# maropu/hivemall

Measured on AMD Instinct MI355X. Metric: rows/sec (node) FFM on Criteo-shaped sparse at 1/2/4/8 MI355X; logloss parity, higher is better.
Workload: dtype fp32; 1 GPU; global_batch=262144, seq_len=39, nnz_per_row=39, fields=explicit, parallelism=dp1, mix_every=10, state=fp32 V, fp32 AdaGrad accumulator per (feature, field) slot (fp32 math), state_layout=packed, reload=False, mixed_bytes_per_mix=671088656, mix_overlapped=False, mix_wire=bf16_delta, early_ramp_warmup_steps=1, linear_steps=side-table, resident_batches=8

## Files before the change

csrc/kernels/ffm.hip:

```cpp
#include <type_traits>

#include "common.h"

namespace {

struct FFMParams {
    int B, F;
    int num_features, num_fields, Kp;
    int classification;
    int train;
    int use_linear, use_bias, norm;
    int reload;
    int gstride;
    int vpad;
    int tail16;
    int gfstride;
    int sstride;
    int fstride;
    long long vfe;
    uint32_t seed;
    float eta0, eps, lambda_v;
    float alpha, beta, lambda1, lambda2;
    float min_target, max_target;
    const uint8_t* hot;
// ... 791 lines not shown
            defer_row(P, row);
        } else if (P.train) {
            const float ks = kappa * scale * scale;
            const f2 eps = {P.eps, P.eps};
            const f2 meta = {-P.eta0, -P.eta0};
            uint32_t hrow = (P.seed ^ ((uint32_t)row * 0x85EBCA77u)) + tid_h;
            hrow ^= hrow >> 16;
            hrow *= 0x7FEB352Du;
            hrow ^= hrow >> 15;
#pragma unroll
            for (int j = 0; j < NS; ++j) {
                const int s = tid + j * 256;
                const f2 coef = {ks * xab[j], ks * xab[j]};
                f2 o0, o1, g0, g1, p0, p1;
                if constexpr (BF) {
                    const uint2 pv = s_t[s < FF ? s : 0];
                    o0 = bf2_to_f2(q[j].x); o1 = bf2_to_f2(q[j].y);
                    g0 = bf2_to_f2(q[j].z); g1 = bf2_to_f2(q[j].w);
                    p0 = bf2_to_f2(pv.x);   p1 = bf2_to_f2(pv.y);
                } else {
                    const float4 pv = s_t[s < FF ? s : 0];
                    o0 = f2{qv[j].x, qv[j].y}; o1 = f2{qv[j].z, qv[j].w};
                    g0 = f2{qg[j].x, qg[j].y}; g1 = f2{qg[j].z, qg[j].w};
                    p0 = f2{pv.x, pv.y};       p1 = f2{pv.z, pv.w};
                }
                const float lj = (live >> j & 1u) ? P.lambda_v : 0.f;
                const f2 lamj = {lj, lj};
                const f2 d0 = coef * p0 + lamj * o0, d1 = coef * p1 + lamj * o1;
                g0 = g0 + d0 * d0;
                g1 = g1 + d1 * d1;
                const f2 t0 = g0 + eps, t1 = g1 + eps;
                const f2 r0 = {__builtin_amdgcn_rsqf(t0.x), __builtin_amdgcn_rsqf(t0.y)};
                const f2 r1 = {__builtin_amdgcn_rsqf(t1.x), __builtin_amdgcn_rsqf(t1.y)};
                o0 = o0 + meta * d0 * r0;
                o1 = o1 + meta * d1 * r1;
                if constexpr (!BF) {
                    if (wr >> j & 1u) {
                        *reinterpret_cast<float4*>(vg + off[j]) = make_float4(o0.x, o0.y, o1.x, o1.y);
                        *reinterpret_cast<float4*>(vg + off[j] + 16u) = make_float4(g0.x, g0.y, g1.x, g1.y);
                    }
                    continue;
                }
                const uint32_t h = rotl32(hrow, 5 * j + 1) ^ (0x9E3779B9u * (uint32_t)(j + 1));
                const uint4 st = make_uint4(pack_sr_hi(o0, h, rotl32(h, 16)),
                                            pack_sr_hi(o1, rotl32(h, 8), rotl32(h, 24)),
                                            pack_sr_hi(g0, rotl32(h, 4), rotl32(h, 20)),
                                            pack_sr_hi(g1, rotl32(h, 12), rotl32(h, 28)));
                if (wr >> j & 1u) *reinterpret_cast<uint4*>(vg + off[j]) = st;
            }
            if (wave == 0 && lane < F) {
                const int pi = s_m[cur][lane].x;
                if (pi >= 0) {
                    for (int f = P.num_fields; f < (int)nfld; ++f) {
                        *reinterpret_cast<uint4*>(vg + ((uint32_t)pi * nfld + (uint32_t)f) * SLOT_B) = make_uint4(0u, 0u, 0u, 0u);
                        if (!BF) *reinterpret_cast<uint4*>(vg + ((uint32_t)pi * nfld + (uint32_t)f) * SLOT_B + 16u) = make_uint4(0u, 0u, 0u, 0u);
                    }
                }
            }
            if (mi >= 0) {
                if (P.use_linear) {
                    const float lz = s_lin[cur][1][lane];
                    const float ln = s_lin[cur][2][lane];
                    const float g = kappa * mx * scale;
                    const float n1 = ln + g * g;
                    const float z1 = lz + g - (sqrtf(n1) - sqrtf(ln)) / P.alpha * lw;
                    LW(wz, mi) = z1;
                    LW(wn, mi) = n1;
                    LW(w, mi) = ftrl_weight(z1, n1, P.alpha, P.beta, P.lambda1, P.lambda2);
                }
            }
            if (P.use_bias && tid == 0) bias_update(P, kappa, bias);
        }
        if (more) dma_lin(nxt);
    }
    __builtin_amdgcn_s_waitcnt(0x0F70);
#undef SA
#undef SB
}


typedef uint32_t u3v_t __attribute__((ext_vector_type(3)));

#define VMCNT_ENC(n) ((((n) & 15) | (((n) >> 4) << 14)) | 0x0F70)
template <int NS, typename OT, int TPB = 256, int ATOM = 0, int KV = 1, int KEEP = 0, int LT = 0>
__global__ __launch_bounds__(TPB) __attribute__((amdgpu_waves_per_eu(TPB / 128))) void ffm_pipe_sg32_kernel(
    FFMParams P, const int32_t* __restrict__ idx, const int32_t* __restrict__ fld,
    const float* __restrict__ val, const float* __restrict__ y, void* __restrict__ Vt,
    float* __restrict__ Gt, float* __restrict__ w, float* __restrict__ wz, float* __restrict__ wn,
    float* __restrict__ bias, float* __restrict__ pred_out, float* __restrict__ loss_out)
{
    __shared__ __attribute__((aligned(16))) float4 s_rv[NS * TPB * KV];
    __shared__ __attribute__((aligned(16))) float s_rg[NS * TPB];
    __shared__ __attribute__((aligned(16))) float4 s_t[NS * TPB * KV];
    __shared__ __attribute__((aligned(16))) int4 s_m[2][48];
    __shared__ __attribute__((aligned(16))) int s_mr[2][3][48];
    __shared__ __attribute__((aligned(16))) float s_lin[2][3][48];
    __shared__ __attribute__((aligned(16))) float4 s_lin4[2][48];
    __shared__ float s_red[TPB / 64 + 2];
    __shared__ int s_rep[TPB / 64];
    __shared__ float s_bias[4];
    __shared__ float s_bcur[2];
    __shared__ float2 s_hd[LT ? HD_SIZE : 1];
    __shared__ __attribute__((aligned(16))) float4 s_hacc[LT ? 2 : 1][48];
    __shared__ __attribute__((aligned(16))) int s_nh[LT ? 2 : 1][48];
    const int F = P.F;
    const int FF = F * F;
    const int tid = threadIdx.x, wave = tid >> 6, lane = tid & 63;
    constexpr int W_META = 1, W_LIN = 2, W_DMA = 3;
    const OT vfs = (OT)P.fstride * (16u * KV);
    const OT gfs = (OT)P.gstride * 4u;
    const int G = (int)gridDim.x;
    const int bid = (int)blockIdx.x;
    char* vb = reinterpret_cast<char*>(Vt);
    char* gb = reinterpret_cast<char*>(Gt);
    const bool latom = ATOM == 0 && !LT && P.lin_atomic == 1 && G > 1;
    if constexpr (LT != 0) {
        for (int t = tid; t < HD_SIZE; t += TPB) s_hd[t] = make_float2(0.f, 0.f);
    }
    int nh = -1, kh = -1;

    int ab[NS];
#pragma unroll
    for (int j = 0; j < NS; ++j) {
        const int s = tid + j * TPB;
        ab[j] = s < FF ? (s / F) | ((s % F) << 8) : 0;
    }
#define SA(j) (ab[j] & 0xFF)
#define SB(j) (ab[j] >> 8)

    auto dma_meta = [&](int bf, int row) {
        if (wave == W_DMA && lane < F && row < P.B) {
            const size_t o = (size_t)row * F + lane;
            __builtin_amdgcn_global_load_lds((glb_ptr_t)(idx + o), (lds_ptr_t)&s_mr[bf][0][0], 4, 0, 0);
            if (fld) __builtin_amdgcn_global_load_lds((glb_ptr_t)(fld + o), (lds_ptr_t)&s_mr[bf][1][0], 4, 0, 0);
            if (val) __builtin_amdgcn_global_load_lds((glb_ptr_t)(val + o), (lds_ptr_t)&s_mr[bf][2][0], 4, 0, 0);
        }
    };
    auto publish_meta = [&](int bf) {
        if (wave == W_META) {
            float sq = 0.f;
            if (lane < F) {
                int ri = s_mr[bf][0][lane];
                int rf = fld ? s_mr[bf][1][lane] : lane;
                float rx = val ? __int_as_float(s_mr[bf][2][lane]) : 1.f;
                if (ri < 0 || ri >= P.num_features || rf < 0 || rf >= P.num_fields) { ri = -1; rx = 0.f; rf = 0; }
                const int hb = ((ATOM == 2 || (latom && P.lin_atomic >= 2)) && ri >= 0) ? (int)P.hot[ri] : 0;
                s_m[bf][lane] = make_int4(ri, rf, __float_as_int(rx), hb);
                sq = rx * rx;
            }
            const float tot = hm::wave_sum_uniform(sq);
            if (lane == 0) s_red[TPB / 64 + bf] = (P.norm && tot > 0.f) ? rsqrtf(tot) : 1.f;
        }
    };
    auto slot = [&](int bf, int j, OT& ov, OT& og, float& xab) -> uint32_t {
        const int4 ma = s_m[bf][SA(j)], mb = s_m[bf][SB(j)];
        const bool ok = (ma.x | mb.x) >= 0 && tid + j * TPB < FF;
        const bool live = ok && SA(j) != SB(j);
        const OT i = ok ? (OT)(uint32_t)ma.x : (OT)0, f = ok ? (OT)(uint32_t)mb.y : (OT)0;
        ov = i * vfs + f * (16u * KV);
        og = i * gfs + f * 4u;
        xab = live ? __int_as_float(ma.z) * __int_as_float(mb.z) : 0.f;
        return live ? 1u : (ok ? 2u : 0u);
    };
    OT kov[KEEP ? NS : 1], kog[KEEP ? NS : 1], nov[KEEP ? NS : 1], nog[KEEP ? NS : 1];
    float kxab[KEEP ? NS : 1], nxab[KEEP ? NS : 1];
    uint32_t klive = 0u, kwr = 0u, nlive = 0u, nwr = 0u;
    int krep = 0, nrep = 0;
    auto dma_slots = [&](int bf) {
        if constexpr (KEEP) { nlive = 0u; nwr = 0u; nrep = 0; }
#pragma unroll
        for (int j = 0; j < NS; ++j) {
            OT ov, og;
            float xab;
            const uint32_t k = slot(bf, j, ov, og, xab);
            if constexpr (KEEP) {
                nov[j] = ov;
                nog[j] = og;
                nxab[j] = xab;
                nlive |= (k & 1u) << j;
                nwr |= (uint32_t)(k != 0u) << j;
                if (P.defer) nrep |= (int)slot_repeats(SA(j), SB(j), s_m[bf][SA(j)], s_m[bf][SB(j)]);
            }
#pragma unroll
            for (int q = 0; q < KV; ++q)
                __builtin_amdgcn_global_load_lds((glb_ptr_t)(vb + ov + 16u * q),
                                                 (lds_ptr_t)(s_rv + (q * NS + j) * TPB + wave * 64), 16, 0, 0);
            __builtin_amdgcn_global_load_lds((glb_ptr_t)(gb + og), (lds_ptr_t)(s_rg + j * TPB + wave * 64), 4, 0, 0);
        }
    };
    auto keep_rotate = [&]() {
        if constexpr (KEEP) {
#pragma unroll
            for (int j = 0; j < NS; ++j) { kov[j] = nov[j]; kog[j] = nog[j]; kxab[j] = nxab[j]; }
            klive = nlive; kwr = nwr; krep = nrep;
        }
    };
    const int nlin = (P.use_linear && P.lin_defer) ? ((P.lpack || !P.train) ? 1 + (LT != 0) : 3) : 0;
    auto dma_lin = [&](int bf) {
        if (P.use_linear && wave == W_LIN && lane < F) {
            const int i = max(s_m[bf][lane].x, 0);
            if (P.lpack) {
                __builtin_amdgcn_global_load_lds((glb_ptr_t)&LW(w, i), (lds_ptr_t)&s_lin4[bf][0], 16, 0, 0);
                if constexpr (LT != 0)
                    __builtin_amdgcn_global_load_lds((glb_ptr_t)(P.hacc + HACC_STRIDE * max(nh, 0)), (lds_ptr_t)&s_hacc[bf][0], 16, 0, 0);
                return;
            }
            __builtin_amdgcn_global_load_lds((glb_ptr_t)&LW(w, i), (lds_ptr_t)&s_lin[bf][0][0], 4, 0, 0);
            if (P.train) {
                __builtin_amdgcn_global_load_lds((glb_ptr_t)&LW(wz, i), (lds_ptr_t)&s_lin[bf][1][0], 4, 0, 0);
                __builtin_amdgcn_global_load_lds((glb_ptr_t)&LW(wn, i), (lds_ptr_t)&s_lin[bf][2][0], 4, 0, 0);
            }
        }
    };

    int row = bid;
    if (row >= P.B) return;
    if (tid == 0) { s_bcur[0] = 0.f; s_bcur[1] = 0.f; }
    dma_meta(0, row);
    __builtin_amdgcn_s_waitcnt(0x0F70);
    bar_raw();
    publish_meta(0);
    bar_raw();
    dma_slots(0);
    keep_rotate();
    if constexpr (LT != 0) {
        if (wave == W_LIN && lane < F) nh = s_m[0][lane].x >= 0 ? P.hidx[s_m[0][lane].x] : -1;
    }
    dma_lin(0);
    kh = nh;
    dma_meta(1, row + G);

    float4 fv[NS][KV];
    float fg[NS];
    OT fo[NS];
    uint32_t fwd = 0u;
    const bool bsh = P.use_bias && P.bias_sh;
    int bit = 0;
    float bz = 0.f, bn = 0.f;
    if (bsh && wave == W_META && lane < P.bias_s) {
        bz = __hip_atomic_load(P.bias_sh + lane * 32, __ATOMIC_RELAXED, __HIP_MEMORY_SCOPE_AGENT);
        bn = __hip_atomic_load(P.bias_sh + lane * 32 + 1, __ATOMIC_RELAXED, __HIP_MEMORY_SCOPE_AGENT);
    }
    for (int cur = 0; row < P.B; row += G, cur ^= 1) {
        const int nxt = cur ^ 1;
        const bool more = row + G < P.B;
        if (wave == W_LIN && nlin == 3) __builtin_amdgcn_s_waitcnt(0x0F73);
        else if (wave == W_LIN && nlin == 2) __builtin_amdgcn_s_waitcnt(0x0F72);
        else if (wave == W_LIN && nlin == 1) __builtin_amdgcn_s_waitcnt(0x0F71);
        else __builtin_amdgcn_s_waitcnt(0x0F70);
        bar_raw();
        const bool bre = bsh && bit > 0 && (bit % P.bias_every) == 0;
        float nbz = bz, nbn = bn;
        if (bre && wave == W_META && lane < P.bias_s) {
            nbz = __hip_atomic_load(P.bias_sh + lane * 32, __ATOMIC_RELAXED, __HIP_MEMORY_SCOPE_AGENT);
            nbn = __hip_atomic_load(P.bias_sh + lane * 32 + 1, __ATOMIC_RELAXED, __HIP_MEMORY_SCOPE_AGENT);
        }
        if constexpr (LT != 0) {
            if (more && wave == W_LIN && lane < F) {
                const int ri = s_mr[nxt][0][lane];
                __builtin_amdgcn_global_load_lds((glb_ptr_t)(P.hidx + (ri >= 0 && ri < P.num_features ? ri : 0)),
                                                 (lds_ptr_t)&s_nh[nxt][0], 4, 0, 0);
            }
        }
        float cg[NS];
#pragma unroll
        for (int j = 0; j < NS; ++j) {
            cg[j] = s_rg[j * TPB + tid];
            float4 v[KV];
#pragma unroll
            for (int q = 0; q < KV; ++q) v[q] = s_rv[(q * NS + j) * TPB + tid];
            if (fwd >> j & 1u) {
                bool same;
                if constexpr (KEEP) {
                    same = (kwr >> j & 1u) && kov[j] == fo[j];
                } else {
                    OT ov, og;
                    float xq;
                    same = slot(cur, j, ov, og, xq) != 0u && ov == fo[j];
                }
                if (same) {
#pragma unroll
                    for (int q = 0; q < KV; ++q) v[q] = fv[j][q];
                    cg[j] = fg[j];
                }
            }
            if (tid + j * TPB < FF) {
#pragma unroll
                for (int q = 0; q < KV; ++q) s_t[(SB(j) * F + SA(j)) * KV + q] = v[q];
            }
        }
        fwd = 0u;
        if (more) publish_meta(nxt);
        bar_raw();
        if (more) {
            dma_slots(nxt);
            dma_meta(cur, row + 2 * G);
        }
        const float scale = s_red[TPB / 64 + cur];
        int mi = -1;
        float mx = 0.f, lw = 0.f;
        int hot = 0;
        float hz = 0.f, hn = 0.f;
        if (wave == W_LIN && nlin) {
            if (more) __builtin_amdgcn_s_waitcnt(VMCNT_ENC((KV + 1) * NS));
            else __builtin_amdgcn_s_waitcnt(0x0F70);
        }
        if (wave == W_LIN && lane < F) {
            const int4 m = s_m[cur][lane];
            mi = m.x;
            mx = __int_as_float(m.z);
            lw = P.lpack ? s_lin4[cur][lane].x : s_lin[cur][0][lane];
            if (latom) lw = lin_w(P, s_lin4[cur][lane]);
            if constexpr (LT != 0) {
                if (P.hacc_on && mi >= 0 && kh >= 0) {
                    const float4 a = s_hacc[cur][lane];
                    const float2 d = s_hd[kh];
                    hz = a.x + d.x;
                    hn = a.y + d.y;
                    hot = 1;
                    lw = hn > 0.f ? ftrl_weight(hz, hn, P.alpha, P.beta, P.lambda1, P.lambda2) : lw;
                }
            }
        }
        uint32_t live = 0u, wr = 0u;
        float xab[NS];
        float4 kpv[KEEP >= 2 ? NS : 1][KEEP >= 2 ? KV : 1], kcv[KEEP >= 2 ? NS : 1][KEEP >= 2 ? KV : 1];
        float part = 0.f;
        int rep = 0;
        if constexpr (KEEP) { live = klive; wr = kwr; rep = krep; }
#pragma unroll
        for (int j = 0; j < NS; ++j) {
            if constexpr (KEEP) {
                xab[j] = kxab[j];
            } else {
                OT ov, og;
                const uint32_t k = slot(cur, j, ov, og, xab[j]);
                live |= (k & 1u) << j;
                wr |= (uint32_t)(k != 0u) << j;
                if (P.defer) rep |= (int)slot_repeats(SA(j), SB(j), s_m[cur][SA(j)], s_m[cur][SB(j)]);
            }
            const int s = tid + j * TPB;
            float dot = 0.f;
#pragma unroll
            for (int q = 0; q < KV; ++q) {
                const float4 pv = s_t[(s < FF ? s : 0) * KV + q];
                const float4 cv = s_t[(SB(j) * F + SA(j)) * KV + q];
                if constexpr (KEEP >= 2) { kpv[j][q] = pv; kcv[j][q] = cv; }
                dot += cv.x * pv.x + cv.y * pv.y + cv.z * pv.z + cv.w * pv.w;
            }
            part += dot * xab[j];
        }
        part *= 0.5f * scale * scale;
        part += lw * mx * scale;
        part = hm::wave_sum_uniform(part);
        const int wrep = __any(rep);
        if (bsh && wave == W_META) {
            const float z = hm::wave_sum_uniform(bz) + s_bcur[0], n = hm::wave_sum_uniform(bn) + s_bcur[1];
            if (lane == 0) { s_bias[0] = ftrl_weight(z, n, P.alpha, P.beta, 0.f, 0.f); s_bias[1] = z; s_bias[2] = n; }
        }
        if (lane == 0) { s_red[wave] = part; s_rep[wave] = wrep; }
        bar_raw();
        float p = 0.f;
        int rdup = 0;
#pragma unroll
        for (int q = 0; q < TPB / 64; ++q) { p += s_red[q]; rdup |= s_rep[q]; }
        if (P.use_bias) p += bsh ? s_bias[0] : bias_w0(P, bias);
        const float kappa = row_loss(P, row, p, y, pred_out, loss_out);

        if (bre && tid == 0) { s_bcur[0] = 0.f; s_bcur[1] = 0.f; }
        if (P.train && rdup && P.defer) {
            defer_row(P, row);
        } else if (P.train) {
            const float ks = kappa * scale * scale;
#pragma unroll
            for (int j = 0; j < NS; ++j) {
                if (!(wr >> j & 1u)) continue;
                OT ov, og;
                if constexpr (KEEP) {
                    ov = kov[j];
                    og = kog[j];
                } else {
                    float xj;
                    slot(cur, j, ov, og, xj);
                }
                const int s = tid + j * TPB;
                const float c = ks * xab[j];
                const float lj = (live >> j & 1u) ? P.lambda_v : 0.f;
                const f2 cc = {c, c}, ll = {lj, lj};
                f2 o0[KV], o1[KV], d0[KV], d1[KV];
                float gs = cg[j];
#pragma unroll
                for (int q = 0; q < KV; ++q) {
                    const float4 pv = KEEP >= 2 ? kpv[j][q] : s_t[s * KV + q];
                    const float4 cv = KEEP >= 2 ? kcv[j][q] : s_t[(SB(j) * F + SA(j)) * KV + q];
                    o0[q] = f2{cv.x, cv.y};
                    o1[q] = f2{cv.z, cv.w};
                    const f2 p0 = f2{pv.x, pv.y}, p1 = f2{pv.z, pv.w};
                    d0[q] = cc * p0 + ll * o0[q];
                    d1[q] = cc * p1 + ll * o1[q];
                    gs = (((gs + d0[q].x * d0[q].x) + d0[q].y * d0[q].y) + d1[q].x * d1[q].x) + d1[q].y * d1[q].y;
                }
                const float r = __builtin_amdgcn_rsqf(gs + P.eps) * -P.eta0;
                const f2 rr = {r, r};
#pragma unroll
                for (int q = 0; q < KV; ++q) {
                    const f2 n0 = o0[q] + rr * d0[q], n1 = o1[q] + rr * d1[q];
                    fv[j][q] = make_float4(n0.x, n0.y, n1.x, n1.y);
                }
                fg[j] = gs;
                fo[j] = ov;
                fwd |= 1u << j;
                if (ATOM == 1 || (ATOM == 2 && s_m[cur][SA(j)].w != 0)) {
                    if (live >> j & 1u) {
                        float* vp = reinterpret_cast<float*>(vb + ov);
#pragma unroll
                        for (int q = 0; q < KV; ++q) {
                            const f2 e0 = rr * d0[q], e1 = rr * d1[q];
                            atomicAdd(vp + 4 * q + 0, e0.x);
                            atomicAdd(vp + 4 * q + 1, e0.y);
                            atomicAdd(vp + 4 * q + 2, e1.x);
                            atomicAdd(vp + 4 * q + 3, e1.y);
                        }
                        atomicAdd(reinterpret_cast<float*>(gb + og), gs - cg[j]);
                    }
                    continue;
                }
#pragma unroll
                for (int q = 0; q < KV; ++q) *reinterpret_cast<float4*>(vb + ov + 16u * q) = fv[j][q];
                *reinterpret_cast<float*>(gb + og) = fg[j];
            }
            if (mi >= 0) {
                if (P.use_linear) {
                    const float lz = hot ? hz : (P.lpack ? s_lin4[cur][lane].y : s_lin[cur][1][lane]);
                    const float ln = hot ? hn : (P.lpack ? s_lin4[cur][lane].z : s_lin[cur][2][lane]);
                    const float g = kappa * mx * scale;
                    const float n1 = ln + g * g;
                    const float z1 = lz + g - (sqrtf(n1) - sqrtf(ln)) / P.alpha * lw;
                    const float w1 = ftrl_weight(z1, n1, P.alpha, P.beta, P.lambda1, P.lambda2);
                    if (LT && hot) {
                        const float2 d = s_hd[kh];
                        s_hd[kh] = make_float2(d.x + (g - (sqrtf(n1) - sqrtf(ln)) / P.alpha * lw), d.y + g * g);
                    } else if (ATOM == 1 || (ATOM == 2 && s_m[cur][lane].w != 0)) {
                        atomicAdd(&LW(wz, mi), z1 - lz);
                        atomicAdd(&LW(wn, mi), g * g);
                        LW(w, mi) = w1;
                    } else if (latom && (P.lin_atomic == 1 || (P.lin_atomic == 2) == (s_m[cur][lane].w != 0))) {
                        lin_add(P, w, mi, g, ln, n1, lw);
                    } else if (P.lpack) {
                        *reinterpret_cast<float4*>(&LW(w, mi)) = make_float4(w1, z1, n1, s_lin4[cur][lane].w);
                    } else {
                        LW(wz, mi) = z1;
                        LW(wn, mi) = n1;
                        LW(w, mi) = w1;
                    }
                }
            }
            if (P.use_bias && tid == 0) {
                if (bsh) bias_update_sh(P, kappa, s_bias[1], s_bias[2], P.bias_sh + (blockIdx.x % P.bias_s) * 32, s_bcur);
                else bias_update(P, kappa, bias);
            }
        }
        if constexpr (LT != 0) {
            if (more && wave == W_LIN && lane < F) nh = s_nh[nxt][lane];
        }
        if (more) dma_lin(nxt);
        kh = nh;
        keep_rotate();
        bz = nbz;
        bn = nbn;
        ++bit;
    }
    __builtin_amdgcn_s_waitcnt(0x0F70);
    if constexpr (LT != 0) {
        bar_raw();
        if (P.hacc_on)
            for (int t = tid; t < 2 * P.nhot; t += TPB) {
                const float2 d = s_hd[t >> 1];
                if (d.y != 0.f || d.x != 0.f) atomicAdd(P.hacc + HACC_STRIDE * (t >> 1) + (t & 1), (t & 1) ? d.y : d.x);
            }
    }
#undef SA
#undef SB
}

template <int NS, typename OT, int KEEP = 0, int LT = 0>
__global__ __launch_bounds__(256) __attribute__((amdgpu_waves_per_eu(4))) void ffm_pipe_sg12_kernel(
    FFMParams P, const int32_t* __restrict__ idx, const int32_t* __restrict__ fld,
    const float* __restrict__ val, const float* __restrict__ y, void* __restrict__ Vt,
    float* __restrict__ w, float* __restrict__ wz, float* __restrict__ wn,
    float* __restrict__ bias, float* __restrict__ pred_out, float* __restrict__ loss_out)
{
    __shared__ __attribute__((aligned(16))) uint32_t s_raw[NS * 256 * 4];
    __shared__ __attribute__((aligned(16))) uint2 s_t[NS * 256];
    __shared__ __attribute__((aligned(16))) int4 s_m[2][48];
    __shared__ __attribute__((aligned(16))) int s_mr[2][3][48];
    __shared__ __attribute__((aligned(16))) float s_lin[2][3][48];
    __shared__ __attribute__((aligned(16))) float4 s_lin4[2][48];
    __shared__ float s_red[8];
    __shared__ int s_rep[4];
    __shared__ float s_bias[4];
    __shared__ float s_bcur[2];
    __shared__ float2 s_hd[LT ? HD12_SIZE : 1];
    __shared__ __attribute__((aligned(16))) float4 s_hacc[LT ? 2 : 1][48];
    __shared__ __attribute__((aligned(16))) int s_nh[LT ? 2 : 1][48];
    const int F = P.F;
    const int FF = F * F;
    const int tid = threadIdx.x, wave = tid >> 6, lane = tid & 63;
    constexpr int W_META = 1, W_LIN = 2, W_DMA = 3;
    const OT bs = (OT)P.gstride * 4u;
    const int G = gridDim.x;
    char* vb = reinterpret_cast<char*>(Vt);
    const bool latom = !LT && P.lin_atomic == 1 && G > 1;
    if constexpr (LT != 0) {
        for (int t = tid; t < HD12_SIZE; t += 256) s_hd[t] = make_float2(0.f, 0.f);
    }
    int nh = -1, kh = -1;
    const bool lin_in_tail = reinterpret_cast<const char*>(w) == vb + (size_t)P.vpad * 12;
    typedef uint32_t u3v __attribute__((ext_vector_type(3)));

    int ab[NS];
#pragma unroll
    for (int j = 0; j < NS; ++j) {
        const int s = tid + j * 256;
        ab[j] = s < FF ? (s / F) | ((s % F) << 8) : 0;
    }
#define SA(j) (ab[j] & 0xFF)
#define SB(j) (ab[j] >> 8)
    const uint32_t tid_h = (uint32_t)tid * 0x9E3779B1u;

    auto dma_meta = [&](int bf, int row) {
        if (wave == W_DMA && lane < F && row < P.B) {
            const size_t o = (size_t)row * F + lane;
            __builtin_amdgcn_global_load_lds((glb_ptr_t)(idx + o), (lds_ptr_t)&s_mr[bf][0][0], 4, 0, 0);
            if (fld) __builtin_amdgcn_global_load_lds((glb_ptr_t)(fld + o), (lds_ptr_t)&s_mr[bf][1][0], 4, 0, 0);
            if (val) __builtin_amdgcn_global_load_lds((glb_ptr_t)(val + o), (lds_ptr_t)&s_mr[bf][2][0], 4, 0, 0);
        }
    };
    auto publish_meta = [&](int bf) {
        if (wave == W_META) {
            float sq = 0.f;
            if (lane < F) {
                int ri = s_mr[bf][0][lane];
                int rf = fld ? s_mr[bf][1][lane] : lane;
                float rx = val ? __int_as_float(s_mr[bf][2][lane]) : 1.f;
                if (ri < 0 || ri >= P.num_features || rf < 0 || rf >= P.num_fields) { ri = -1; rx = 0.f; rf = 0; }
                s_m[bf][lane] = make_int4(ri, rf, __float_as_int(rx), 0);
                sq = rx * rx;
            }
            const float tot = hm::wave_sum_uniform(sq);
            if (lane == 0) s_red[4 + bf] = (P.norm && tot > 0.f) ? rsqrtf(tot) : 1.f;
        }
    };
    auto slot = [&](int bf, int j, OT& off, float& xab) -> uint32_t {
        const int4 ma = s_m[bf][SA(j)], mb = s_m[bf][SB(j)];
        const bool ok = (ma.x | mb.x) >= 0 && tid + j * 256 < FF;
        const bool live = ok && SA(j) != SB(j);
        off = ok ? (OT)(uint32_t)ma.x * bs + (OT)(uint32_t)mb.y * 12u : (OT)0;
        xab = live ? __int_as_float(ma.z) * __int_as_float(mb.z) : 0.f;
        return live ? 1u : (ok ? 2u : 0u);
    };
    OT koff[KEEP ? NS : 1], noff[KEEP ? NS : 1];
    float kxab[KEEP ? NS : 1], nxab[KEEP ? NS : 1];
    uint32_t klive = 0u, kwr = 0u, nlive = 0u, nwr = 0u;
    int krep = 0, nrep = 0;
    auto dma_slots = [&](int bf) {
// ... 245 lines not shown
    }
    __builtin_amdgcn_s_waitcnt(0x0F70);
    if constexpr (LT != 0) {
        bar_raw();
        if (P.hacc_on)
            for (int t = tid; t < 2 * P.nhot; t += 256) {
                const float2 d = s_hd[t >> 1];
                if (d.y != 0.f || d.x != 0.f) atomicAdd(P.hacc + HACC_STRIDE * (t >> 1) + (t & 1), (t & 1) ? d.y : d.x);
            }
    }
#undef SA
#undef SB
}


int default_blocks(int B, int grid, int cap = 256 * 8 * 4) {
    return grid > 0 ? grid : (B < cap ? B : cap);
}

template <bool BF>
int dispatch_lean(const FFMParams& P, const int32_t* idx, const int32_t* fld, const float* val,
                  const float* y, void* VG, float* w, float* wz, float* wn, float* bias,
                  float* pred, float* loss, int grid, int variant, hipStream_t stream) {
    const size_t slot_b = BF ? 16 : 32;
    if (P.Kp != 4 || P.F > 45) return -1;
    if ((size_t)P.num_features * (size_t)P.fstride * slot_b >= ((size_t)1 << 32)) return -1;
    const size_t meta = (size_t)P.F * 16 + 16 * 4;
    const size_t sh = (size_t)P.F * P.F * (BF ? 8 : 16) + meta;
    const int need = (P.F * P.F + 255) / 256;
    const int blocks = default_blocks(P.B, grid);
    if (blocks <= 0) return 0;
    if ((BF && variant != 2) || (!BF && variant == 3)) {
#define HM_PIPE(NSV) hipLaunchKernelGGL((ffm_pipe_kernel<NSV, BF>), dim3(blocks), dim3(256), 0, stream, P, idx, \
                                        fld, val, y, VG, w, wz, wn, bias, pred, loss)
        if (need <= 2) { HM_PIPE(2); }
        else if (need <= 4) { HM_PIPE(4); }
        else if (need <= 6) { HM_PIPE(6); }
        else { HM_PIPE(8); }
#undef HM_PIPE
        HM_LAUNCH_RET();
    }
#define HM_LEAN(NSV)                                                                                \
    hipLaunchKernelGGL((ffm_lean_kernel<BF, NSV>), dim3(blocks), dim3(256), sh, stream, P, idx, fld, \
                       val, y, VG, w, wz, wn, bias, pred, loss)
    if (need <= 2) HM_LEAN(2);
    else if (need <= 4) HM_LEAN(4);
    else if (need <= 6) HM_LEAN(6);
    else HM_LEAN(8);
#undef HM_LEAN
    HM_LAUNCH_RET();
}

__global__ __launch_bounds__(256) void ffm_hacc_kernel(FFMParams P, float* __restrict__ w, int dir) {
    const int h = blockIdx.x * 256 + threadIdx.x;
    if (h >= P.nhot) return;
    float4* rp = reinterpret_cast<float4*>(&LW(w, P.hot_id[h]));
    float4* ap = reinterpret_cast<float4*>(P.hacc + HACC_STRIDE * h);
    const float4 r = *rp;
    if (dir == 0) {
        *ap = make_float4(r.y, r.z, 0.f, 0.f);
    } else {
        const float4 a = *ap;
        const float nw = a.y > 0.f ? ftrl_weight(a.x, a.y, P.alpha, P.beta, P.lambda1, P.lambda2) : r.x;
        *rp = make_float4(nw, a.x, a.y, r.w);
    }
}

__global__ __launch_bounds__(256) void ffm_lin_derive_kernel(FFMParams P, float* __restrict__ w) {
    const int i = blockIdx.x * 256 + threadIdx.x;
    if (i >= P.num_features) return;
    const float4 r = *reinterpret_cast<const float4*>(&LW(w, i));
    if (r.z > 0.f) LW(w, i) = ftrl_weight(r.y, r.z, P.alpha, P.beta, P.lambda1, P.lambda2);
}

int dispatch_sg12(const FFMParams& P, const int32_t* idx, const int32_t* fld, const float* val,
                  const float* y, void* VG, float* w, float* wz, float* wn, float* bias,
                  float* pred, float* loss, int grid, int variant, hipStream_t stream) {
    if (P.Kp != 4 || P.F > 45) return -1;
    const bool wide = (size_t)P.num_features * (size_t)P.gstride * 4 >= ((size_t)1 << 32);
    const int need = (P.F * P.F + 255) / 256;
    int blocks = default_blocks(P.B, grid, 256 * 8 * 8);
    if (blocks <= 0) return 0;
    FFMParams Q = P;
    Q.hacc_on = P.lin_atomic == 4 && P.nhot <= HD12_SIZE && blocks > 1 && !wide && variant != 9 && variant != 10;
    if (Q.hacc_on && grid <= 0) blocks = default_blocks(P.B, grid, HACC_GRID12);
    if (Q.hacc_on) {
        hipLaunchKernelGGL(ffm_hacc_kernel, dim3((P.nhot + 255) / 256), dim3(256), 0, stream, Q, w, 0);
        HM_LAUNCH_RET_IF_ERR();
    }
#define HM_P12(NSV) do { \
        if (wide) hipLaunchKernelGGL((ffm_pipe_sg12_kernel<NSV, uint64_t>), dim3(blocks), dim3(256), 0, stream, \
                                     P, idx, fld, val, y, VG, w, wz, wn, bias, pred, loss); \
        else if (Q.hacc_on) hipLaunchKernelGGL((ffm_pipe_sg12_kernel<NSV, uint32_t, 2, 1>), dim3(blocks), dim3(256), 0, \
                                               stream, Q, idx, fld, val, y, VG, w, wz, wn, bias, pred, loss); \
        else if (variant == 9) hipLaunchKernelGGL((ffm_pipe_sg12_kernel<NSV, uint32_t>), dim3(blocks), dim3(256), 0, \
                                                  stream, P, idx, fld, val, y, VG, w, wz, wn, bias, pred, loss); \
        else if (variant == 10) hipLaunchKernelGGL((ffm_pipe_sg12_kernel<NSV, uint32_t, 1>), dim3(blocks), dim3(256), 0, \
                                                   stream, P, idx, fld, val, y, VG, w, wz, wn, bias, pred, loss); \
        else hipLaunchKernelGGL((ffm_pipe_sg12_kernel<NSV, uint32_t, 2>), dim3(blocks), dim3(256), 0, stream, \
                                P, idx, fld, val, y, VG, w, wz, wn, bias, pred, loss); } while (0)
    if (need <= 2) { HM_P12(2); }
    else if (need <= 4) { HM_P12(4); }
    else if (need <= 6) { HM_P12(6); }
    else { HM_P12(8); }
#undef HM_P12
    if (Q.hacc_on) {
        HM_LAUNCH_RET_IF_ERR();
        hipLaunchKernelGGL(ffm_hacc_kernel, dim3((P.nhot + 255) / 256), dim3(256), 0, stream, Q, w, 1);
    }
    HM_LAUNCH_RET();
}

int dispatch_sg32(const FFMParams& P, const int32_t* idx, const int32_t* fld, const float* val,
                  const float* y, void* V, float* G, float* w, float* wz, float* wn, float* bias,
                  float* pred, float* loss, int grid, int variant, hipStream_t stream) {
    if ((P.Kp != 4 && P.Kp != 8) || P.F > 45 || P.vpad <= 0) return -1;
    const bool wide = (size_t)P.num_features * (size_t)P.fstride * (size_t)(P.Kp * 4) >= ((size_t)1 << 32) ||
                      (size_t)P.num_features * (size_t)P.gstride * 4 >= ((size_t)1 << 32);
    if (P.Kp == 8) {
        if (variant == 8) return -1;
        const int need = (P.F * P.F + 511) / 512;
        int blocks = default_blocks(P.B, grid);
        if (blocks <= 0) return 0;
        FFMParams Q = P;
        Q.hacc_on = P.lin_atomic == 4 && blocks > 1 && !wide && variant != 6 && variant != 9;
        if (Q.hacc_on && grid <= 0) blocks = default_blocks(P.B, grid, HACC_GRID);
        if (Q.hacc_on) {
            hipLaunchKernelGGL(ffm_hacc_kernel, dim3((P.nhot + 255) / 256), dim3(256), 0, stream, Q, w, 0);
            HM_LAUNCH_RET_IF_ERR();
        }
#define HM_P32K8(NSV) do { \
        if (wide) hipLaunchKernelGGL((ffm_pipe_sg32_kernel<NSV, uint64_t, 512, 0, 2>), dim3(blocks), dim3(512), 0, stream, \
                                     P, idx, fld, val, y, V, G, w, wz, wn, bias, pred, loss); \
        else if (Q.hacc_on) hipLaunchKernelGGL((ffm_pipe_sg32_kernel<NSV, uint32_t, 512, 0, 2, 1, 1>), dim3(blocks), \
                                               dim3(512), 0, stream, Q, idx, fld, val, y, V, G, w, wz, wn, \
                                               bias, pred, loss); \
        else if (variant == 6) hipLaunchKernelGGL((ffm_pipe_sg32_kernel<NSV, uint32_t, 512, 1, 2>), dim3(blocks), \
                                                  dim3(512), 0, stream, P, idx, fld, val, y, V, G, w, wz, wn, \
                                                  bias, pred, loss); \
        else if (variant == 9) hipLaunchKernelGGL((ffm_pipe_sg32_kernel<NSV, uint32_t, 512, 0, 2>), dim3(blocks), \
                                                  dim3(512), 0, stream, P, idx, fld, val, y, V, G, w, wz, wn, \
                                                  bias, pred, loss); \
        else hipLaunchKernelGGL((ffm_pipe_sg32_kernel<NSV, uint32_t, 512, 0, 2, 1>), dim3(blocks), dim3(512), 0, stream, \
                                P, idx, fld, val, y, V, G, w, wz, wn, bias, pred, loss); } while (0)
        if (need <= 2) { HM_P32K8(2); }
        else if (need <= 3) { HM_P32K8(3); }
        else { HM_P32K8(4); }
#undef HM_P32K8
        if (Q.hacc_on) {
            HM_LAUNCH_RET_IF_ERR();
            hipLaunchKernelGGL(ffm_hacc_kernel, dim3((P.nhot + 255) / 256), dim3(256), 0, stream, Q, w, 1);
        }
        HM_LAUNCH_RET();
    }
    const int need = (P.F * P.F + 255) / 256;
    int blocks = default_blocks(P.B, grid);
    if (blocks <= 0) return 0;
    FFMParams Q = P;
    Q.hacc_on = P.lin_atomic == 4 && blocks > 1 && !wide && variant != 6 && variant != 8 && variant != 9 && variant != 10;
    if (Q.hacc_on && grid <= 0) blocks = default_blocks(P.B, grid, HACC_GRID);
    if (Q.hacc_on) {
        hipLaunchKernelGGL(ffm_hacc_kernel, dim3((P.nhot + 255) / 256), dim3(256), 0, stream, Q, w, 0);
        HM_LAUNCH_RET_IF_ERR();
    }
#define HM_P32(NSV) do { \
        if (wide) hipLaunchKernelGGL((ffm_pipe_sg32_kernel<NSV, uint64_t>), dim3(blocks), dim3(256), 0, stream, \
                                     P, idx, fld, val, y, V, G, w, wz, wn, bias, pred, loss); \
        else if (variant == 6) hipLaunchKernelGGL((ffm_pipe_sg32_kernel<NSV, uint32_t, 256, 1>), dim3(blocks), \
                                                  dim3(256), 0, stream, P, idx, fld, val, y, V, G, w, wz, wn, \
                                                  bias, pred, loss); \
        else if (variant == 8 && P.hot) hipLaunchKernelGGL((ffm_pipe_sg32_kernel<NSV, uint32_t, 256, 2>), dim3(blocks), \
                                                  dim3(256), 0, stream, P, idx, fld, val, y, V, G, w, wz, wn, \
                                                  bias, pred, loss); \
        else if (variant == 9) hipLaunchKernelGGL((ffm_pipe_sg32_kernel<NSV, uint32_t>), dim3(blocks), dim3(256), 0, \
                                                  stream, P, idx, fld, val, y, V, G, w, wz, wn, bias, pred, loss); \
        else if (variant == 10) hipLaunchKernelGGL((ffm_pipe_sg32_kernel<NSV, uint32_t, 256, 0, 1, 1>), dim3(blocks), \
                                                   dim3(256), 0, stream, P, idx, fld, val, y, V, G, w, wz, wn, \
                                                   bias, pred, loss); \
        else if (Q.hacc_on) hipLaunchKernelGGL((ffm_pipe_sg32_kernel<NSV, uint32_t, 256, 0, 1, 2, 1>), dim3(blocks), \
                                               dim3(256), 0, stream, Q, idx, fld, val, y, V, G, w, wz, wn, \
                                               bias, pred, loss); \
        else hipLaunchKernelGGL((ffm_pipe_sg32_kernel<NSV, uint32_t, 256, 0, 1, 2>), dim3(blocks), dim3(256), 0, stream, \
                                P, idx, fld, val, y, V, G, w, wz, wn, bias, pred, loss); } while (0)
    if (need <= 2) { HM_P32(2); }
    else if (need <= 4) { HM_P32(4); }
    else if (need <= 6) { HM_P32(6); }
    else { HM_P32(8); }
#undef HM_P32
    if (Q.hacc_on) {
        HM_LAUNCH_RET_IF_ERR();
        hipLaunchKernelGGL(ffm_hacc_kernel, dim3((P.nhot + 255) / 256), dim3(256), 0, stream, Q, w, 1);
    }
    HM_LAUNCH_RET();
}

template <int KC, bool BF, bool SG>
int launch_ffm(const FFMParams& P, const int32_t* idx, const int32_t* fld, const float* val,
               const float* y, void* V, void* G, float* w, float* wz, float* wn, float* bias,
               float* pred, float* loss, int grid, hipStream_t stream) {
    const size_t meta = (size_t)6 * P.F * 4 + 16 * 4;
    const size_t stage = (size_t)P.F * P.F * KC * (BF ? 8 : 16);
    const bool use_stage = stage + meta <= 64 * 1024;
    const int blocks = default_blocks(P.B, grid);
    if (blocks <= 0) return 0;
    if (use_stage) {
        hipLaunchKernelGGL((ffm_row_kernel<KC, true, BF, SG>), dim3(blocks), dim3(256), stage + meta, stream,
                           P, idx, fld, val, y, V, G, w, wz, wn, bias, pred, loss);
    } else {
        hipLaunchKernelGGL((ffm_row_kernel<KC, false, BF, SG>), dim3(blocks), dim3(256), meta, stream,
                           P, idx, fld, val, y, V, G, w, wz, wn, bias, pred, loss);
    }
    HM_LAUNCH_RET();
}

template <bool BF, bool SG>
int launch_generic(const FFMParams& P, const int32_t* idx, const int32_t* fld, const float* val,
                   const float* y, void* V, void* G, float* w, float* wz, float* wn, float* bias,
                   float* pred, float* loss, int grid, hipStream_t stream) {
    switch (P.Kp / 4) {
        case 1: return launch_ffm<1, BF, SG>(P, idx, fld, val, y, V, G, w, wz, wn, bias, pred, loss, grid, stream);
        case 2: return launch_ffm<2, BF, SG>(P, idx, fld, val, y, V, G, w, wz, wn, bias, pred, loss, grid, stream);
        case 3: return launch_ffm<3, BF, SG>(P, idx, fld, val, y, V, G, w, wz, wn, bias, pred, loss, grid, stream);
        case 4: return launch_ffm<4, BF, SG>(P, idx, fld, val, y, V, G, w, wz, wn, bias, pred, loss, grid, stream);
        case 8: return launch_ffm<8, BF, SG>(P, idx, fld, val, y, V, G, w, wz, wn, bias, pred, loss, grid, stream);
        default: return (int)hipErrorInvalidValue;
    }
}

template <bool BF>
int dispatch(const FFMParams& P, const int32_t* idx, const int32_t* fld, const float* val,
             const float* y, void* V, void* G, float* w, float* wz, float* wn, float* bias,
             float* pred, float* loss, int grid, int packed, int slot_g, int variant, hipStream_t stream,
             int* fast) {
    *fast = 1;
    if (slot_g) {
        if (P.gfstride == 3) {
            if (!BF) return (int)hipErrorInvalidValue;
            const int rc = variant == 1 ? -1 : dispatch_sg12(P, idx, fld, val, y, V, w, wz, wn, bias, pred, loss, grid, variant, stream);
            if (rc != -1) return rc;
            *fast = 0;
            return launch_generic<true, true>(P, idx, fld, val, y, V, G, w, wz, wn, bias, pred, loss, grid, stream);
        }
        if (variant != 1 && !BF && P.gfstride == 1) {
            const int rc = dispatch_sg32(P, idx, fld, val, y, V, reinterpret_cast<float*>(G), w, wz, wn,
                                         bias, pred, loss, grid, variant, stream);
            if (rc != -1) return rc;
        }
        *fast = 0;
        return launch_generic<BF, true>(P, idx, fld, val, y, V, G, w, wz, wn, bias, pred, loss, grid, stream);
    }
// ... 114 lines not shown
```

Baseline: 84.49 million rows/s.

## Add specialized SG32 training kernel variant with compile-time config and precomputed offsets

Adds a CFG template flag that builds a training-specialized ffm_pipe_sg32_kernel in which runtime parameter checks (train, linear, lpack, fld/val, bias) become compile-time constants. Slot indexing is precomputed into packed bitfields with a validity mask, and the per-feature V/G row offset is cached in the metadata int4 so the V and G addresses share a base. The kernel's own V vector is kept in registers instead of re-read from LDS, and the wave index is made scalar via readfirstlane. The host dispatches this variant when the config matches, which trades extra template instantiations and register pressure for fewer runtime branches and less address math. hacc_on now also requires lin_defer.

```diff
diff --git a/csrc/kernels/ffm.hip b/csrc/kernels/ffm.hip
--- a/csrc/kernels/ffm.hip
+++ b/csrc/kernels/ffm.hip
@@ -897,13 +897,33 @@
 typedef uint32_t u3v_t __attribute__((ext_vector_type(3)));
 
 #define VMCNT_ENC(n) ((((n) & 15) | (((n) >> 4) << 14)) | 0x0F70)
-template <int NS, typename OT, int TPB = 256, int ATOM = 0, int KV = 1, int KEEP = 0, int LT = 0>
+template <bool PIN>
+__device__ __forceinline__ float dot4_products_rounded(float4 c, float4 p) {
+    float m0 = c.x * p.x, m1 = c.y * p.y, m2 = c.z * p.z, m3 = c.w * p.w;
+    if constexpr (PIN) asm("" : "+v"(m0), "+v"(m1), "+v"(m2), "+v"(m3));
+    return m0 + m1 + m2 + m3;
+}
+
+constexpr int SG32_TRAIN = 1;
+
+template <int NS, typename OT, int TPB = 256, int ATOM = 0, int KV = 1, int KEEP = 0, int LT = 0, int CFG = 0>
 __global__ __launch_bounds__(TPB) __attribute__((amdgpu_waves_per_eu(TPB / 128))) void ffm_pipe_sg32_kernel(
     FFMParams P, const int32_t* __restrict__ idx, const int32_t* __restrict__ fld,
     const float* __restrict__ val, const float* __restrict__ y, void* __restrict__ Vt,
     float* __restrict__ Gt, float* __restrict__ w, float* __restrict__ wz, float* __restrict__ wn,
     float* __restrict__ bias, float* __restrict__ pred_out, float* __restrict__ loss_out)
 {
+    constexpr bool SPEC = (CFG & SG32_TRAIN) != 0;
+    static_assert(!SPEC || (ATOM == 0 && KV == 1 && KEEP >= 2 && sizeof(OT) == 4 && TPB == 256),
+                  "SG32_TRAIN: the default fp32 k <= 4 training launch only");
+#define c_train (SPEC || P.train)
+#define c_linear (SPEC || P.use_linear)
+#define c_lpack (SPEC || P.lpack)
+#define c_ldefer (SPEC || P.lin_defer)
+#define c_bias (!SPEC && P.use_bias)
+#define c_fld (SPEC || fld)
+#define c_val (SPEC || val)
+#define c_hacc (SPEC ? LT != 0 : P.hacc_on)
     __shared__ __attribute__((aligned(16))) float4 s_rv[NS * TPB * KV];
     __shared__ __attribute__((aligned(16))) float s_rg[NS * TPB];
     __shared__ __attribute__((aligned(16))) float4 s_t[NS * TPB * KV];
@@ -920,7 +940,8 @@
     __shared__ __attribute__((aligned(16))) int s_nh[LT ? 2 : 1][48];
     const int F = P.F;
     const int FF = F * F;
-    const int tid = threadIdx.x, wave = tid >> 6, lane = tid & 63;
+    const int tid = threadIdx.x, lane = tid & 63;
+    const int wave = SPEC ? __builtin_amdgcn_readfirstlane(tid >> 6) : tid >> 6;
     constexpr int W_META = 1, W_LIN = 2, W_DMA = 3;
     const OT vfs = (OT)P.fstride * (16u * KV);
     const OT gfs = (OT)P.gstride * 4u;
@@ -928,27 +949,35 @@
     const int bid = (int)blockIdx.x;
     char* vb = reinterpret_cast<char*>(Vt);
     char* gb = reinterpret_cast<char*>(Gt);
-    const bool latom = ATOM == 0 && !LT && P.lin_atomic == 1 && G > 1;
+    const bool latom = !SPEC && ATOM == 0 && !LT && P.lin_atomic == 1 && G > 1;
     if constexpr (LT != 0) {
         for (int t = tid; t < HD_SIZE; t += TPB) s_hd[t] = make_float2(0.f, 0.f);
     }
     int nh = -1, kh = -1;
 
     int ab[NS];
+    uint32_t okm = 0u;
 #pragma unroll
     for (int j = 0; j < NS; ++j) {
         const int s = tid + j * TPB;
-        ab[j] = s < FF ? (s / F) | ((s % F) << 8) : 0;
-    }
-#define SA(j) (ab[j] & 0xFF)
-#define SB(j) (ab[j] >> 8)
+        if constexpr (SPEC) {
+            const int a = s < FF ? s / F : 0, b = s < FF ? s % F : 0;
+            ab[j] = (a << 4) | (b << 10) | ((s < FF ? b * F + a : s) << 16);
+            okm |= (uint32_t)(s >= FF) << j | (uint32_t)(s >= FF || a == b) << (8 + j) | (uint32_t)(a < b) << (16 + j);
+        } else {
+            ab[j] = s < FF ? (s / F) | ((s % F) << 8) : 0;
+        }
+    }
+#define SA(j) (SPEC ? (ab[j] >> 4) & 0x3F : ab[j] & 0xFF)
+#define SB(j) (SPEC ? (ab[j] >> 10) & 0x3F : ab[j] >> 8)
+#define ST(j) (SPEC ? ab[j] >> 16 : (SB(j) * F + SA(j)) * KV)
 
     auto dma_meta = [&](int bf, int row) {
         if (wave == W_DMA && lane < F && row < P.B) {
             const size_t o = (size_t)row * F + lane;
             __builtin_amdgcn_global_load_lds((glb_ptr_t)(idx + o), (lds_ptr_t)&s_mr[bf][0][0], 4, 0, 0);
-            if (fld) __builtin_amdgcn_global_load_lds((glb_ptr_t)(fld + o), (lds_ptr_t)&s_mr[bf][1][0], 4, 0, 0);
-            if (val) __builtin_amdgcn_global_load_lds((glb_ptr_t)(val + o), (lds_ptr_t)&s_mr[bf][2][0], 4, 0, 0);
+            if (c_fld) __builtin_amdgcn_global_load_lds((glb_ptr_t)(fld + o), (lds_ptr_t)&s_mr[bf][1][0], 4, 0, 0);
+            if (c_val) __builtin_amdgcn_global_load_lds((glb_ptr_t)(val + o), (lds_ptr_t)&s_mr[bf][2][0], 4, 0, 0);
         }
     };
     auto publish_meta = [&](int bf) {
@@ -956,10 +985,11 @@
             float sq = 0.f;
             if (lane < F) {
                 int ri = s_mr[bf][0][lane];
-                int rf = fld ? s_mr[bf][1][lane] : lane;
-                float rx = val ? __int_as_float(s_mr[bf][2][lane]) : 1.f;
+                int rf = c_fld ? s_mr[bf][1][lane] : lane;
+                float rx = c_val ? __int_as_float(s_mr[bf][2][lane]) : 1.f;
                 if (ri < 0 || ri >= P.num_features || rf < 0 || rf >= P.num_fields) { ri = -1; rx = 0.f; rf = 0; }
-                const int hb = ((ATOM == 2 || (latom && P.lin_atomic >= 2)) && ri >= 0) ? (int)P.hot[ri] : 0;
+                const int hb = SPEC ? (ri >= 0 ? (int)((uint32_t)ri * (uint32_t)vfs) : 0)
+                                    : ((ATOM == 2 || (latom && P.lin_atomic >= 2)) && ri >= 0) ? (int)P.hot[ri] : 0;
                 s_m[bf][lane] = make_int4(ri, rf, __float_as_int(rx), hb);
                 sq = rx * rx;
             }
@@ -983,6 +1013,29 @@
     int krep = 0, nrep = 0;
     auto dma_slots = [&](int bf) {
         if constexpr (KEEP) { nlive = 0u; nwr = 0u; nrep = 0; }
+        if constexpr (SPEC) {
+            uint32_t eq = 0u;
+#pragma unroll
+            for (int j = 0; j < NS; ++j) {
+                const int4 ma = s_m[bf][SA(j)], mb = s_m[bf][SB(j)];
+                const int both = ma.x | mb.x;
+                const bool ok = (both | (int)(okm << (31 - j))) >= 0;
+                const bool live = (both | (int)(okm << (23 - j))) >= 0;
+                const OT ib = ok ? (OT)(uint32_t)ma.w : (OT)0, f = ok ? (OT)(uint32_t)mb.y : (OT)0;
+                OT f4 = f * 4u;
+                asm("" : "+v"(f4));
+                nov[j] = ib + f * 16u;
+                nog[j] = ib + f4;
+                nxab[j] = live ? __int_as_float(ma.z) * __int_as_float(mb.z) : 0.f;
+                nwr |= (uint32_t)ok << j;
+                eq |= (uint32_t)(ma.x == mb.x || ma.y == mb.y) << j;
+                __builtin_amdgcn_global_load_lds((glb_ptr_t)(vb + nov[j]), (lds_ptr_t)(s_rv + j * TPB + wave * 64), 16, 0, 0);
+                __builtin_amdgcn_global_load_lds((glb_ptr_t)(gb + nog[j]), (lds_ptr_t)(s_rg + j * TPB + wave * 64), 4, 0, 0);
+            }
+            nlive = nwr & ~(okm >> 8);
+            if (P.defer) nrep = (int)(eq & nwr & (okm >> 16));
+            return;
+        }
 #pragma unroll
         for (int j = 0; j < NS; ++j) {
             OT ov, og;
@@ -1010,18 +1063,18 @@
             klive = nlive; kwr = nwr; krep = nrep;
         }
     };
-    const int nlin = (P.use_linear && P.lin_defer) ? ((P.lpack || !P.train) ? 1 + (LT != 0) : 3) : 0;
+    const int nlin = (c_linear && c_ldefer) ? ((c_lpack || !c_train) ? 1 + (LT != 0) : 3) : 0;
     auto dma_lin = [&](int bf) {
-        if (P.use_linear && wave == W_LIN && lane < F) {
+        if (c_linear && wave == W_LIN && lane < F) {
             const int i = max(s_m[bf][lane].x, 0);
-            if (P.lpack) {
+            if (c_lpack) {
                 __builtin_amdgcn_global_load_lds((glb_ptr_t)&LW(w, i), (lds_ptr_t)&s_lin4[bf][0], 16, 0, 0);
                 if constexpr (LT != 0)
                     __builtin_amdgcn_global_load_lds((glb_ptr_t)(P.hacc + HACC_STRIDE * max(nh, 0)), (lds_ptr_t)&s_hacc[bf][0], 16, 0, 0);
                 return;
             }
             __builtin_amdgcn_global_load_lds((glb_ptr_t)&LW(w, i), (lds_ptr_t)&s_lin[bf][0][0], 4, 0, 0);
-            if (P.train) {
+            if (c_train) {
                 __builtin_amdgcn_global_load_lds((glb_ptr_t)&LW(wz, i), (lds_ptr_t)&s_lin[bf][1][0], 4, 0, 0);
                 __builtin_amdgcn_global_load_lds((glb_ptr_t)&LW(wn, i), (lds_ptr_t)&s_lin[bf][2][0], 4, 0, 0);
             }
@@ -1049,7 +1102,7 @@
     float fg[NS];
     OT fo[NS];
     uint32_t fwd = 0u;
-    const bool bsh = P.use_bias && P.bias_sh;
+    const bool bsh = c_bias && P.bias_sh;
     int bit = 0;
     float bz = 0.f, bn = 0.f;
     if (bsh && wave == W_META && lane < P.bias_s) {
@@ -1059,6 +1112,7 @@
     for (int cur = 0; row < P.B; row += G, cur ^= 1) {
         const int nxt = cur ^ 1;
         const bool more = row + G < P.B;
+        if constexpr (SPEC) asm volatile("" : "+v"(okm));
         if (wave == W_LIN && nlin == 3) __builtin_amdgcn_s_waitcnt(0x0F73);
         else if (wave == W_LIN && nlin == 2) __builtin_amdgcn_s_waitcnt(0x0F72);
         else if (wave == W_LIN && nlin == 1) __builtin_amdgcn_s_waitcnt(0x0F71);
@@ -1078,6 +1132,7 @@
             }
         }
         float cg[NS];
+        float4 own[SPEC ? NS : 1];
 #pragma unroll
         for (int j = 0; j < NS; ++j) {
             cg[j] = s_rg[j * TPB + tid];
@@ -1099,9 +1154,12 @@
                     cg[j] = fg[j];
                 }
             }
-            if (tid + j * TPB < FF) {
-#pragma unroll
-                for (int q = 0; q < KV; ++q) s_t[(SB(j) * F + SA(j)) * KV + q] = v[q];
+            if constexpr (SPEC) {
+                s_t[ST(j)] = v[0];
+                own[j] = v[0];
+            } else if (tid + j * TPB < FF) {
+#pragma unroll
+                for (int q = 0; q < KV; ++q) s_t[ST(j) + q] = v[q];
             }
         }
         fwd = 0u;
@@ -1124,10 +1182,10 @@
             const int4 m = s_m[cur][lane];
             mi = m.x;
             mx = __int_as_float(m.z);
-            lw = P.lpack ? s_lin4[cur][lane].x : s_lin[cur][0][lane];
+            lw = c_lpack ? s_lin4[cur][lane].x : s_lin[cur][0][lane];
             if (latom) lw = lin_w(P, s_lin4[cur][lane]);
             if constexpr (LT != 0) {
-                if (P.hacc_on && mi >= 0 && kh >= 0) {
+                if (c_hacc && mi >= 0 && kh >= 0) {
                     const float4 a = s_hacc[cur][lane];
                     const float2 d = s_hd[kh];
                     hz = a.x + d.x;
@@ -1158,10 +1216,12 @@
             float dot = 0.f;
 #pragma unroll
             for (int q = 0; q < KV; ++q) {
-                const float4 pv = s_t[(s < FF ? s : 0) * KV + q];
-                const float4 cv = s_t[(SB(j) * F + SA(j)) * KV + q];
+                const float4 pv = s_t[(SPEC || s < FF ? s : 0) * KV + q];
+                float4 cv;
+                if constexpr (SPEC) cv = own[j];
+                else cv = s_t[ST(j) + q];
                 if constexpr (KEEP >= 2) { kpv[j][q] = pv; kcv[j][q] = cv; }
-                dot += cv.x * pv.x + cv.y * pv.y + cv.z * pv.z + cv.w * pv.w;
+                dot += dot4_products_rounded<SPEC>(cv, pv);
             }
             part += dot * xab[j];
         }
@@ -1179,13 +1239,13 @@
         int rdup = 0;
 #pragma unroll
         for (int q = 0; q < TPB / 64; ++q) { p += s_red[q]; rdup |= s_rep[q]; }
-        if (P.use_bias) p += bsh ? s_bias[0] : bias_w0(P, bias);
+        if (c_bias) p += bsh ? s_bias[0] : bias_w0(P, bias);
         const float kappa = row_loss(P, row, p, y, pred_out, loss_out);
 
         if (bre && tid == 0) { s_bcur[0] = 0.f; s_bcur[1] = 0.f; }
-        if (P.train && rdup && P.defer) {
+        if (c_train && rdup && P.defer) {
             defer_row(P, row);
-        } else if (P.train) {
+        } else if (c_train) {
             const float ks = kappa * scale * scale;
 #pragma unroll
             for (int j = 0; j < NS; ++j) {
@@ -1207,7 +1267,7 @@
 #pragma unroll
                 for (int q = 0; q < KV; ++q) {
                     const float4 pv = KEEP >= 2 ? kpv[j][q] : s_t[s * KV + q];
-                    const float4 cv = KEEP >= 2 ? kcv[j][q] : s_t[(SB(j) * F + SA(j)) * KV + q];
+                    const float4 cv = KEEP >= 2 ? kcv[j][q] : s_t[ST(j) + q];
                     o0[q] = f2{cv.x, cv.y};
                     o1[q] = f2{cv.z, cv.w};
                     const f2 p0 = f2{pv.x, pv.y}, p1 = f2{pv.z, pv.w};
@@ -1245,9 +1305,9 @@
                 *reinterpret_cast<float*>(gb + og) = fg[j];
             }
             if (mi >= 0) {
-                if (P.use_linear) {
-                    const float lz = hot ? hz : (P.lpack ? s_lin4[cur][lane].y : s_lin[cur][1][lane]);
-                    const float ln = hot ? hn : (P.lpack ? s_lin4[cur][lane].z : s_lin[cur][2][lane]);
+                if (c_linear) {
+                    const float lz = hot ? hz : (c_lpack ? s_lin4[cur][lane].y : s_lin[cur][1][lane]);
+                    const float ln = hot ? hn : (c_lpack ? s_lin4[cur][lane].z : s_lin[cur][2][lane]);
                     const float g = kappa * mx * scale;
                     const float n1 = ln + g * g;
                     const float z1 = lz + g - (sqrtf(n1) - sqrtf(ln)) / P.alpha * lw;
@@ -1261,7 +1321,7 @@
                         LW(w, mi) = w1;
                     } else if (latom && (P.lin_atomic == 1 || (P.lin_atomic == 2) == (s_m[cur][lane].w != 0))) {
                         lin_add(P, w, mi, g, ln, n1, lw);
-                    } else if (P.lpack) {
+                    } else if (c_lpack) {
                         *reinterpret_cast<float4*>(&LW(w, mi)) = make_float4(w1, z1, n1, s_lin4[cur][lane].w);
                     } else {
                         LW(wz, mi) = z1;
@@ -1270,7 +1330,7 @@
                     }
                 }
             }
-            if (P.use_bias && tid == 0) {
+            if (c_bias && tid == 0) {
                 if (bsh) bias_update_sh(P, kappa, s_bias[1], s_bias[2], P.bias_sh + (blockIdx.x % P.bias_s) * 32, s_bcur);
                 else bias_update(P, kappa, bias);
             }
@@ -1288,7 +1348,7 @@
     __builtin_amdgcn_s_waitcnt(0x0F70);
     if constexpr (LT != 0) {
         bar_raw();
-        if (P.hacc_on)
+        if (c_hacc)
             for (int t = tid; t < 2 * P.nhot; t += TPB) {
                 const float2 d = s_hd[t >> 1];
                 if (d.y != 0.f || d.x != 0.f) atomicAdd(P.hacc + HACC_STRIDE * (t >> 1) + (t & 1), (t & 1) ? d.y : d.x);
@@ -1296,6 +1356,15 @@
     }
 #undef SA
 #undef SB
+#undef ST
+#undef c_train
+#undef c_linear
+#undef c_lpack
+#undef c_ldefer
+#undef c_bias
+#undef c_fld
+#undef c_val
+#undef c_hacc
 }
 
 template <int NS, typename OT, int KEEP = 0, int LT = 0>
@@ -1707,7 +1776,7 @@
     int blocks = default_blocks(P.B, grid, 256 * 8 * 8);
     if (blocks <= 0) return 0;
     FFMParams Q = P;
-    Q.hacc_on = P.lin_atomic == 4 && P.nhot <= HD12_SIZE && blocks > 1 && !wide && variant != 9 && variant != 10;
+    Q.hacc_on = P.lin_atomic == 4 && P.lin_defer && P.nhot <= HD12_SIZE && blocks > 1 && !wide && variant != 9 && variant != 10;
     if (Q.hacc_on && grid <= 0) blocks = default_blocks(P.B, grid, HACC_GRID12);
     if (Q.hacc_on) {
         hipLaunchKernelGGL(ffm_hacc_kernel, dim3((P.nhot + 255) / 256), dim3(256), 0, stream, Q, w, 0);
@@ -1748,7 +1817,7 @@
         int blocks = default_blocks(P.B, grid);
         if (blocks <= 0) return 0;
         FFMParams Q = P;
-        Q.hacc_on = P.lin_atomic == 4 && blocks > 1 && !wide && variant != 6 && variant != 9;
+        Q.hacc_on = P.lin_atomic == 4 && P.lin_defer && blocks > 1 && !wide && variant != 6 && variant != 9;
         if (Q.hacc_on && grid <= 0) blocks = default_blocks(P.B, grid, HACC_GRID);
         if (Q.hacc_on) {
             hipLaunchKernelGGL(ffm_hacc_kernel, dim3((P.nhot + 255) / 256), dim3(256), 0, stream, Q, w, 0);
@@ -1782,15 +1851,25 @@
     int blocks = default_blocks(P.B, grid);
     if (blocks <= 0) return 0;
     FFMParams Q = P;
-    Q.hacc_on = P.lin_atomic == 4 && blocks > 1 && !wide && variant != 6 && variant != 8 && variant != 9 && variant != 10;
+    Q.hacc_on = P.lin_atomic == 4 && P.lin_defer && blocks > 1 && !wide && variant != 6 && variant != 8 &&
+                variant != 9 && variant != 10;
     if (Q.hacc_on && grid <= 0) blocks = default_blocks(P.B, grid, HACC_GRID);
     if (Q.hacc_on) {
         hipLaunchKernelGGL(ffm_hacc_kernel, dim3((P.nhot + 255) / 256), dim3(256), 0, stream, Q, w, 0);
         HM_LAUNCH_RET_IF_ERR();
     }
+    const bool spec = variant == 0 && !wide && P.train && P.use_linear && P.lpack && P.lin_defer &&
+                      !P.use_bias && fld && val && P.lin_atomic != 1 &&
+                      (size_t)P.fstride * 16 == (size_t)P.gstride * 4;
 #define HM_P32(NSV) do { \
         if (wide) hipLaunchKernelGGL((ffm_pipe_sg32_kernel<NSV, uint64_t>), dim3(blocks), dim3(256), 0, stream, \
                                      P, idx, fld, val, y, V, G, w, wz, wn, bias, pred, loss); \
+        else if (spec && Q.hacc_on) hipLaunchKernelGGL((ffm_pipe_sg32_kernel<NSV, uint32_t, 256, 0, 1, 2, 1, SG32_TRAIN>), \
+                                                  dim3(blocks), dim3(256), 0, stream, Q, idx, fld, val, y, V, G, w, wz, \
+                                                  wn, bias, pred, loss); \
+        else if (spec) hipLaunchKernelGGL((ffm_pipe_sg32_kernel<NSV, uint32_t, 256, 0, 1, 2, 0, SG32_TRAIN>), \
+                                          dim3(blocks), dim3(256), 0, stream, P, idx, fld, val, y, V, G, w, wz, wn, \
+                                          bias, pred, loss); \
         else if (variant == 6) hipLaunchKernelGGL((ffm_pipe_sg32_kernel<NSV, uint32_t, 256, 1>), dim3(blocks), \
                                                   dim3(256), 0, stream, P, idx, fld, val, y, V, G, w, wz, wn, \
                                                   bias, pred, loss); \
```

Result: faster. 88.20 million rows/s (median of 6 runs) (+4.4%).
